# spencerkent/vision-transform-codes

Hardware: AMD Instinct MI355X
Metric: patches/sec through 200-iter FISTA + dict update, 1024-atom dict (higher is better)
Workload: dtype f16x3

## Files before the change

### vision-transform-codes_amd/csrc/fc_fused.hip

```cpp
#include "fc_fused.h"
#include "fused_common.h"

#include <stdlib.h>
#include <mutex>
#include <vector>

namespace vtc {

struct FusedParams {
  const float* images;
  const float* init;
  float* codes;
  const uint4* packA[2];
  const uint4* packT[2];
  const float* betas;
  int64_t b;
  int s;
  int num_iters;
  int fista;
  float eta, cutoff;
  const float* eta_dev;
  float lam;
  const float* dscale;
  unsigned long long* stamps;
// ... 201 lines not shown
  {                                                                         \
    const int j_ = (i) + RING;                                              \
    const int sg_ = (j_ < 16) ? (sg) : (((sg) + 1) % (2 * NPH));            \
    const int i_ = (j_ < 16) ? j_ : j_ - 16;                                \
    _Pragma("unroll") for (int part = 0; part < NP; ++part)                 \
        ring[part][(i) % RING] = VTC_LOAD_SEG(part, sg_, i_);               \
  }

  auto step3 = [&](int p, int buf, bool pipe, int sg, auto&& between) {
    uint4 yb_next[NP];
#pragma unroll
    for (int part = 0; part < NP; ++part)
      yb_next[part] = *reinterpret_cast<const uint4*>(
          Yx + (buf * NP + part) * kYxPart + yx_rd);
#pragma unroll
    for (int ks = 0; ks < 8; ++ks) {
      uint4 yb[NP];
#pragma unroll
      for (int part = 0; part < NP; ++part) {
        yb[part] = yb_next[part];
        if (ks + 1 < 8)
          yb_next[part] = *reinterpret_cast<const uint4*>(
              Yx + (buf * NP + part) * kYxPart + yx_rd + 32 * (ks + 1));
      }
#pragma unroll
      for (int nb = 0; nb < 2; ++nb) {
        const int i = 2 * ks + nb;
        uint4 a[NP];
#pragma unroll
        for (int part = 0; part < NP; ++part)
          a[part] = pipe ? ring[part][i % RING] : VTC_LOAD_T(part, p, nb, ks);
        Racc[nb] = mfma16<F16>(a[0], yb[0], Racc[nb]);
        if constexpr (NP == 2) {
          Racc[nb] = mfma16<F16>(a[0], yb[1], Racc[nb]);
          Racc[nb] = mfma16<F16>(a[1], yb[0], Racc[nb]);
        }
        between(i);
        if (pipe) VTC_REFILL(sg, i)
        __builtin_amdgcn_sched_barrier(0);
      }
    }
  };
  auto nothing = [](int) {};

  auto exchange_r = [&]() {
    float v[2][16];
#pragma unroll
    for (int nb = 0; nb < 2; ++nb)
#pragma unroll
      for (int e = 0; e < 16; ++e) {
        v[nb][e] = sub_rn(Racc[nb][e], Xr[nb][e]);
        if (F16) v[nb][e] *= r_scale;
      }
    if (F16) {
      float m = 0.f;
#pragma unroll
      for (int nb = 0; nb < 2; ++nb)
#pragma unroll
        for (int e = 0; e < 16; ++e) m = fmaxf(m, fabsf(v[nb][e]));
      m = fmaxf(m, __shfl_xor(m, 32, 64));
      float f = 1.f;
      if (xr_calls > 0) {
        const float* prev = Stat + ((xr_calls - 1) & 1) * 128;
        const float Mx = fmaxf(fmaxf(prev[r], prev[32 + r]),
                               fmaxf(prev[64 + r], prev[96 + r]));
        if (Mx > 2048.f && Mx < __builtin_inff())
          f = ldexpf(1.f, 9 - ilogbf(Mx));
      }
      if (h == 0) Stat[(xr_calls & 1) * 128 + w * 32 + r] = m * f;
      ++xr_calls;
      if (__any(f != 1.f)) {
#pragma unroll
        for (int p = 0; p < NPH; ++p)
#pragma unroll
          for (int e = 0; e < 16; ++e) Y[p][e] *= f;
#pragma unroll
        for (int p = 0; p < CR; ++p)
#pragma unroll
          for (int e = 0; e < 16; ++e) Cr[p][e] *= f;
#pragma unroll
        for (int pl = 0; pl < L::CL; ++pl)
#pragma unroll
          for (int g = 0; g < 4; ++g) {
            float4* c4 = reinterpret_cast<float4*>(Cst + cst_ln + pl * 16384 +
                                                   g * 1024);
            float4 c = *c4;
            c.x *= f; c.y *= f; c.z *= f; c.w *= f;
            *c4 = c;
          }
#pragma unroll
        for (int nb = 0; nb < 2; ++nb)
#pragma unroll
          for (int e = 0; e < 16; ++e) {
            Xr[nb][e] *= f;
            v[nb][e] *= f;
          }
        cutoff_l *= f;
        inv_sigma_y *= 1.f / f;
      }
    }
#pragma unroll
    for (int nb = 0; nb < 2; ++nb) {
#pragma unroll
      for (int g = 0; g < 4; ++g) {
        const float v4[4] = {v[nb][4 * g], v[nb][4 * g + 1], v[nb][4 * g + 2],
                             v[nb][4 * g + 3]};
        uint2 hi, lo;
        split_packed<F16, 4, NP == 2>(v4, hi, lo);
        char* dst = Rx + rx_wr + 64 * nb + 16 * g;
        *reinterpret_cast<uint2*>(dst) = hi;
        if (NP == 2) *reinterpret_cast<uint2*>(dst + kRxPart) = lo;
      }
    }
#pragma unroll
    for (int nb = 0; nb < 2; ++nb)
#pragma unroll
      for (int e = 0; e < 16; ++e) Racc[nb][e] = 0.f;
    __syncthreads();
  };

  if (warm) {
#pragma unroll
    for (int p = 0; p < NPH; ++p) {
      publish_y(Y[p], p & 1);
      __syncthreads();
      step3(p, p & 1, false, 0, nothing);
    }
  }
  exchange_r();

#pragma unroll
  for (int i = 0; i < RING; ++i)
#pragma unroll
    for (int part = 0; part < NP; ++part)
      ring[part][i] = VTC_LOAD_SEG(part, 0, i);

  const bool fista = P.fista != 0;
  unsigned long long acc_t[5] = {0, 0, 0, 0, 0};
  unsigned long long t0 = 0, t1 = 0;
#define VTC_STAMP(slot)                    \
  if (STAMP) {                             \
    t1 = stamp_now();                      \
    acc_t[slot] += t1 - t0;                \
    t0 = t1;                               \
  }
  if (STAMP) t0 = stamp_now();

  f32x16 Gb[2];
  float4 cold4;
  float cn4[4];

  auto epilogue_elem = [&](int p, int e, const f32x16& Gp, float beta) {
    const int g = e >> 2, k = e & 3;
    if (MODE == 7) {
      const float cn = Y[p][e] + Gp[e];
      Y[p][e] = cn;
      cn4[k] = cn;
      if (k == 3) {
        if (p < CREG) {
#pragma unroll
          for (int q = 0; q < 4; ++q) Cr[p < CREG ? p : 0][4 * g + q] = cn4[q];
        } else {
          *reinterpret_cast<float4*>(Cst + cst_ln + (p - CREG) * 16384 +
                                     g * 1024) =
              make_float4(cn4[0], cn4[1], cn4[2], cn4[3]);
        }
      }
      return;
    }
    if (k == 0) {
      if (p < CREG) {
        cold4 = make_float4(Cr[p < CREG ? p : 0][4 * g + 0],
                            Cr[p < CREG ? p : 0][4 * g + 1],
                            Cr[p < CREG ? p : 0][4 * g + 2],
                            Cr[p < CREG ? p : 0][4 * g + 3]);
      } else {
        cold4 = *reinterpret_cast<const float4*>(
            Cst + cst_ln + (p - CREG) * 16384 + g * 1024);
      }
    }
    const float co = (k == 0) ? cold4.x : (k == 1) ? cold4.y
                   : (k == 2) ? cold4.z : cold4.w;
    const float c = sub_rn(Y[p][e], mul_rn(eta, Gp[e]));
    const float cn = shrink_fast<MODE>(c, cutoff_l);
    Y[p][e] = fista ? add_rn(cn, mul_rn(beta, sub_rn(cn, co))) : cn;
    cn4[k] = cn;
    if (k == 3) {
      if (p < CREG) {
#pragma unroll
        for (int q = 0; q < 4; ++q) Cr[p < CREG ? p : 0][4 * g + q] = cn4[q];
      } else {
        *reinterpret_cast<float4*>(Cst + cst_ln + (p - CREG) * 16384 +
                                   g * 1024) =
            make_float4(cn4[0], cn4[1], cn4[2], cn4[3]);
      }
      const float v4[4] = {Y[p][4 * g], Y[p][4 * g + 1], Y[p][4 * g + 2],
                           Y[p][4 * g + 3]};
      uint2 hi, lo;
      split_packed<F16, 4, NP == 2>(v4, hi, lo);
      char* dst = Yx + (p & 1) * NP * kYxPart + yx_wr + 16 * g;
      *reinterpret_cast<uint2*>(dst) = hi;
      if (NP == 2) *reinterpret_cast<uint2*>(dst + kYxPart) = lo;
    }
  };

  auto step1 = [&](int p, int sg, bool overlap, float beta) {
    f32x16& G = Gb[p & 1];
#pragma unroll
    for (int e = 0; e < 16; ++e) G[e] = 0.f;
    uint4 rb_next[NP];
#pragma unroll
    for (int part = 0; part < NP; ++part)
      rb_next[part] =
          *reinterpret_cast<const uint4*>(Rx + part * kRxPart + rx_rd);
#pragma unroll
    for (int i = 0; i < 16; ++i) {
      uint4 rb[NP];
#pragma unroll
      for (int part = 0; part < NP; ++part) {
        rb[part] = rb_next[part];
        if (i + 1 < 16)
          rb_next[part] = *reinterpret_cast<const uint4*>(
              Rx + part * kRxPart + rx_rd + 32 * (i + 1));
      }
      G = mfma16<F16>(ring[0][i % RING], rb[0], G);
      if constexpr (NP == 2) {
        G = mfma16<F16>(ring[0][i % RING], rb[1], G);
        G = mfma16<F16>(ring[1][i % RING], rb[0], G);
      }
      if (overlap) {
        epilogue_elem(p - 1, i, Gb[(p - 1) & 1], beta);
        __builtin_amdgcn_sched_barrier(0);
      }
      VTC_REFILL(sg, i)
      __builtin_amdgcn_sched_barrier(0);
    }
  };

  for (int it = 0; it < P.num_iters; ++it) {
    const float beta = fista ? P.betas[it] : 0.f;
    step1(0, 0, false, beta);
    VTC_STAMP(0)
#pragma unroll
    for (int p = 0; p < NPH; ++p) {
      if (p + 1 < NPH) {
        step1(p + 1, 2 * p + 1, true, beta);
        VTC_STAMP(0)
      }
      __syncthreads();
      VTC_STAMP(2)
      if (p + 2 == NPH) {
        step3(p, p & 1, true, 2 * p + 2, [&](int i) {
          epilogue_elem(NPH - 1, i, Gb[(NPH - 1) & 1], beta);
          __builtin_amdgcn_sched_barrier(0);
        });
      } else {
        step3(p, p & 1, true, (p + 1 < NPH) ? 2 * p + 2 : 2 * NPH - 1, nothing);
      }
      VTC_STAMP(3)
    }
    exchange_r();
    VTC_STAMP(4)
  }
  if (STAMP && lane == 0) {
#pragma unroll
    for (int k = 0; k < 5; ++k) atomicAdd(P.stamps + k, acc_t[k]);
    atomicAdd(P.stamps + 7, 1ull);
  }
#undef VTC_STAMP

#pragma unroll
  for (int p = 0; p < NPH; ++p) {
#pragma unroll
    for (int g = 0; g < 4; ++g) {
      float4 v;
      if (p < CREG) {
        v = make_float4(Cr[p < CREG ? p : 0][4 * g + 0],
                        Cr[p < CREG ? p : 0][4 * g + 1],
                        Cr[p < CREG ? p : 0][4 * g + 2],
                        Cr[p < CREG ? p : 0][4 * g + 3]);
      } else {
        v = *reinterpret_cast<const float4*>(Cst + cst_ln +
                                             (p - CREG) * 16384 + g * 1024);
      }
      if (F16) {
        v.x *= inv_sigma_y;
        v.y *= inv_sigma_y;
        v.z *= inv_sigma_y;
        v.w *= inv_sigma_y;
      }
      if (live)
        *reinterpret_cast<float4*>(P.codes + patch * s + kPhaseAtoms * p +
                                   32 * w + 8 * g + 4 * h) = v;
    }
  }
#undef VTC_LOAD_A
#undef VTC_LOAD_T
#undef VTC_LOAD_SEG
#undef VTC_REFILL
#undef VTC_SEG_IS_T
#undef VTC_SEG_PHASE
}

template <int NPH, int NP, int MODE, bool F16 = false, bool STAMP = false>
__global__ __launch_bounds__(256, 1) void fused_fista_kernel16(FusedParams P) {
  static_assert(!F16 || NP == 2, "the f16 split exists as three products only");
  using L = FusedLds<NPH, NP>;
  constexpr int CREG = L::CREG;
  constexpr int CR = CREG > 0 ? CREG : 1;
  constexpr int RING = (NP == 1) ? 16 : 8;
  constexpr int NPROD = (NP == 2) ? 3 : 1;
  extern __shared__ __attribute__((aligned(16))) char smem[];
  char* Cst = smem;
  char* Yx = smem + L::cst_bytes;
  char* Rx = Yx + L::yx_bytes;
  float* Stat = reinterpret_cast<float*>(Rx + L::rx_bytes);

  const int tid = threadIdx.x;
  const int lane = tid & 63;
  const int w = __builtin_amdgcn_readfirstlane(tid >> 6);
  const int c = lane & 15, q = lane >> 4;
  int64_t patch[2];
  bool live[2];
#pragma unroll
  for (int n = 0; n < 2; ++n) {
    patch[n] = (int64_t)blockIdx.x * kFP + 16 * n + c;
    live[n] = patch[n] < P.b;
  }
  const int s = P.s;

  const unsigned pack_bytes_total = (unsigned)s * kFN * 2u;
  const unsigned a_wave_off = (unsigned)w * (16u * 64u * 16u);
  const unsigned t_wave_off = (unsigned)(4 * w) * (4u * 64u * 16u);
  __amdgpu_buffer_rsrc_t rsA[NP], rsT[NP];
#pragma unroll
  for (int part = 0; part < NP; ++part) {
    rsA[part] = __builtin_amdgcn_make_buffer_rsrc(
        (void*)((const char*)P.packA[part] + a_wave_off), 0,
        (int)(pack_bytes_total - a_wave_off), 0x00020000);
    rsT[part] = __builtin_amdgcn_make_buffer_rsrc(
        (void*)((const char*)P.packT[part] + t_wave_off), 0,
        (int)(pack_bytes_total - t_wave_off), 0x00020000);
  }
  const unsigned frag_voff = (unsigned)lane * 16u;
#define VTC_LOAD_A(part, p, i) \
  buffer_load16(rsA[part], frag_voff, (unsigned)(((4 * (p)) * 16 + (i)) * 1024))
#define VTC_LOAD_T(part, p, nb, ks) \
  buffer_load16(rsT[part], frag_voff,  \
                (unsigned)((((p) * 16 + (nb)) * 4 + (ks)) * 1024))

  const int swap = ((c >> 2) ^ (c >> 3)) & 1;
  const int rd_chunk = 32 * (q >> 1) + 16 * ((q & 1) ^ swap);
  const int wr_chunk = 16 * ((q >> 1) ^ swap) + 8 * (q & 1);
  const int yx_rd = c * kYxRow + rd_chunk;
  const int yx_wr = c * kYxRow + 64 * w + wr_chunk;
  const int rx_rd = c * kRxRow + rd_chunk;
  const int rx_wr = c * kRxRow + 128 * w + wr_chunk;
  const int cst_ln = w * 4096 + lane * 16;
  constexpr int kYxHalf = 16 * kYxRow, kRxHalf = 16 * kRxRow;

  f32x16 Y[NPH];
  f32x16 Cr[CR];
  f32x4 Xr[4][2];
  f32x4 Racc[4][2];
  uint4 ring[NP][RING];

#pragma unroll
  for (int nb = 0; nb < 4; ++nb) {
#pragma unroll
    for (int n = 0; n < 2; ++n) {
      float4 v = make_float4(0.f, 0.f, 0.f, 0.f);
      if (live[n])
        v = *reinterpret_cast<const float4*>(P.images + patch[n] * kFN + 64 * w +
                                             16 * nb + 4 * q);
      Xr[nb][n][0] = v.x;
      Xr[nb][n][1] = v.y;
      Xr[nb][n][2] = v.z;
      Xr[nb][n][3] = v.w;
    }
  }
  const bool warm = (P.init != nullptr);
#pragma unroll
  for (int p = 0; p < NPH; ++p) {
#pragma unroll
    for (int g = 0; g < 4; ++g) {
      float4 v = make_float4(0.f, 0.f, 0.f, 0.f);
      if (warm && live[g & 1])
        v = *reinterpret_cast<const float4*>(P.init + patch[g & 1] * s +
                                             kPhaseAtoms * p + 32 * w +
                                             16 * (g >> 1) + 4 * q);
      Y[p][4 * g + 0] = v.x;
      Y[p][4 * g + 1] = v.y;
      Y[p][4 * g + 2] = v.z;
      Y[p][4 * g + 3] = v.w;
    }
  }
  float sigma_y[2] = {1.f, 1.f}, inv_sigma_y[2] = {1.f, 1.f};
  float sigma_d = 1.f, inv_sigma_d = 1.f;
  if (F16) {
    float sx[2] = {0.f, 0.f}, sy[2] = {0.f, 0.f};
#pragma unroll
    for (int nb = 0; nb < 4; ++nb)
#pragma unroll
      for (int n = 0; n < 2; ++n)
#pragma unroll
        for (int k = 0; k < 4; ++k) sx[n] += Xr[nb][n][k] * Xr[nb][n][k];
    if (warm) {
#pragma unroll
      for (int p = 0; p < NPH; ++p)
#pragma unroll
        for (int e = 0; e < 16; ++e) sy[(e >> 2) & 1] += Y[p][e] * Y[p][e];
    }
    float* red = reinterpret_cast<float*>(Rx);
#pragma unroll
    for (int n = 0; n < 2; ++n) {
      sx[n] += __shfl_xor(sx[n], 16, 64);
      sx[n] += __shfl_xor(sx[n], 32, 64);
      sy[n] += __shfl_xor(sy[n], 16, 64);
      sy[n] += __shfl_xor(sy[n], 32, 64);
      if (q == 0) {
        red[w * 64 + 16 * n + c] = sx[n];
        red[w * 64 + 32 + 16 * n + c] = sy[n];
      }
    }
    __syncthreads();
    float m2[2];
#pragma unroll
    for (int n = 0; n < 2; ++n) {
      float tx = 0.f, ty = 0.f;
#pragma unroll
      for (int v = 0; v < 4; ++v) {
        tx += red[v * 64 + 16 * n + c];
        ty += red[v * 64 + 32 + 16 * n + c];
      }
      m2[n] = fmaxf(tx, ty);
    }
    __syncthreads();
    sigma_d = P.dscale[0];
    inv_sigma_d = P.dscale[1];
#pragma unroll
    for (int n = 0; n < 2; ++n) {
      int e2 = 0;
      if (m2[n] > 0.f && m2[n] < __builtin_inff()) e2 = ilogbf(m2[n]) >> 1;
      e2 = e2 < -60 ? -60 : (e2 > 60 ? 60 : e2);
      sigma_y[n] = ldexpf(1.f, 8 - e2);
      inv_sigma_y[n] = ldexpf(1.f, e2 - 8);
      const float sx_scale = sigma_d * sigma_y[n];
#pragma unroll
      for (int nb = 0; nb < 4; ++nb)
#pragma unroll
        for (int k = 0; k < 4; ++k) Xr[nb][n][k] *= sx_scale;
    }
#pragma unroll
    for (int p = 0; p < NPH; ++p)
#pragma unroll
      for (int e = 0; e < 16; ++e) Y[p][e] *= sigma_y[(e >> 2) & 1];
  }
  float eta = P.eta, cutoff = P.cutoff;
  if (P.eta_dev) {
    eta = *P.eta_dev;
    cutoff = mul_rn(P.lam, eta);
  }
  float cutoff_l[2] = {cutoff, cutoff};
  if (F16) {
    eta = eta * (0.5f * inv_sigma_d);
    cutoff_l[0] = cutoff * sigma_y[0];
    cutoff_l[1] = cutoff * sigma_y[1];
  }
  const float r_scale = F16 ? 2.f * inv_sigma_d : 1.f;
  int xr_calls = 0;
#pragma unroll
  for (int p = 0; p < NPH; ++p) {
#pragma unroll
    for (int g = 0; g < 4; ++g) {
      if (p < CREG) {
#pragma unroll
        for (int k = 0; k < 4; ++k)
          Cr[p < CREG ? p : 0][4 * g + k] = Y[p][4 * g + k];
      } else {
        *reinterpret_cast<float4*>(Cst + cst_ln + (p - CREG) * 16384 +
                                   g * 1024) =
            make_float4(Y[p][4 * g + 0], Y[p][4 * g + 1], Y[p][4 * g + 2],
                        Y[p][4 * g + 3]);
      }
    }
  }
#pragma unroll
  for (int nb = 0; nb < 4; ++nb)
#pragma unroll
    for (int n = 0; n < 2; ++n)
#pragma unroll
      for (int k = 0; k < 4; ++k) Racc[nb][n][k] = 0.f;

  auto publish_group = [&](const f32x16& y, int g, int buf) {
    const float v4[4] = {y[4 * g], y[4 * g + 1], y[4 * g + 2], y[4 * g + 3]};
    uint2 hi, lo;
    split_packed<F16, 4, NP == 2>(v4, hi, lo);
    char* dst = Yx + buf * NP * kYxPart + yx_wr + 32 * (g >> 1) +
                kYxHalf * (g & 1);
    *reinterpret_cast<uint2*>(dst) = hi;
    if (NP == 2) *reinterpret_cast<uint2*>(dst + kYxPart) = lo;
  };

#define VTC_SEG_IS_T(sg) (((sg) >= 2 && ((sg) % 2) == 0) || (sg) == 2 * NPH - 1)
#define VTC_SEG_PHASE(sg)                                        \
  ((sg) == 0 ? 0                                                 \
             : (sg) == 2 * NPH - 1 ? NPH - 1                     \
                                   : ((sg) % 2 ? ((sg) + 1) / 2 : (sg) / 2 - 1))
#define VTC_LOAD_SEG(part, sg, i)                                          \
  (VTC_SEG_IS_T(sg) ? VTC_LOAD_T(part, VTC_SEG_PHASE(sg), (i) & 3, (i) >> 2) \
                    : VTC_LOAD_A(part, VTC_SEG_PHASE(sg), (i)))
#define VTC_REFILL(sg, i)                                                   \
  {                                                                         \
    const int j_ = (i) + RING;                                              \
    const int sg_ = (j_ < 16) ? (sg) : (((sg) + 1) % (2 * NPH));            \
    const int i_ = (j_ < 16) ? j_ : j_ - 16;                                \
    _Pragma("unroll") for (int part = 0; part < NP; ++part)                 \
        ring[part][(i) % RING] = VTC_LOAD_SEG(part, sg_, i_);               \
  }
#define VTC_MFMA_PAIR(acc0, acc1, a, b)                                     \
  _Pragma("unroll") for (int prod = 0; prod < NPROD; ++prod) {              \
    acc0 = mfma_k32<F16>(a[prod == 2], b[0][prod == 1], acc0);              \
    acc1 = mfma_k32<F16>(a[prod == 2], b[1][prod == 1], acc1);              \
  }

  auto step3 = [&](int p, int buf, bool pipe, int sg, auto&& between) {
    uint4 yb[2][NP], yb_next[2][NP];
#pragma unroll
    for (int n = 0; n < 2; ++n)
#pragma unroll
      for (int part = 0; part < NP; ++part)
        yb_next[n][part] = *reinterpret_cast<const uint4*>(
            Yx + (buf * NP + part) * kYxPart + yx_rd + kYxHalf * n);
#pragma unroll
    for (int i = 0; i < 16; ++i) {
      const int ks = i >> 2, nb = i & 3;
      if (nb == 0) {
#pragma unroll
        for (int n = 0; n < 2; ++n)
#pragma unroll
          for (int part = 0; part < NP; ++part) yb[n][part] = yb_next[n][part];
      }
      if (nb < 2 && ks + 1 < 4) {
#pragma unroll
        for (int part = 0; part < NP; ++part)
          yb_next[nb][part] = *reinterpret_cast<const uint4*>(
              Yx + (buf * NP + part) * kYxPart + yx_rd + kYxHalf * nb +
              64 * (ks + 1));
      }
      uint4 a[NP];
#pragma unroll
      for (int part = 0; part < NP; ++part)
        a[part] = pipe ? ring[part][i % RING] : VTC_LOAD_T(part, p, nb, ks);
      VTC_MFMA_PAIR(Racc[nb][0], Racc[nb][1], a, yb)
      between(i);
      if (pipe) VTC_REFILL(sg, i)
      __builtin_amdgcn_sched_barrier(0);
    }
  };
  auto nothing = [](int) {};

  auto exchange_r = [&]() {
    float v[4][2][4];
#pragma unroll
    for (int nb = 0; nb < 4; ++nb)
#pragma unroll
      for (int n = 0; n < 2; ++n)
#pragma unroll
        for (int k = 0; k < 4; ++k) {
          v[nb][n][k] = sub_rn(Racc[nb][n][k], Xr[nb][n][k]);
          if (F16) v[nb][n][k] *= r_scale;
        }
    if (F16) {
      float f[2] = {1.f, 1.f};
#pragma unroll
      for (int n = 0; n < 2; ++n) {
        float m = 0.f;
#pragma unroll
        for (int nb = 0; nb < 4; ++nb)
#pragma unroll
          for (int k = 0; k < 4; ++k) m = fmaxf(m, fabsf(v[nb][n][k]));
        m = fmaxf(m, __shfl_xor(m, 16, 64));
        m = fmaxf(m, __shfl_xor(m, 32, 64));
        const int row = 16 * n + c;
        if (xr_calls > 0) {
          const float* prev = Stat + ((xr_calls - 1) & 1) * 128;
          const float Mx = fmaxf(fmaxf(prev[row], prev[32 + row]),
                                 fmaxf(prev[64 + row], prev[96 + row]));
          if (Mx > 2048.f && Mx < __builtin_inff())
            f[n] = ldexpf(1.f, 9 - ilogbf(Mx));
        }
        if (q == 0) Stat[(xr_calls & 1) * 128 + w * 32 + row] = m * f[n];
      }
      ++xr_calls;
      if (__any(f[0] != 1.f || f[1] != 1.f)) {
#pragma unroll
        for (int p = 0; p < NPH; ++p)
#pragma unroll
          for (int e = 0; e < 16; ++e) Y[p][e] *= f[(e >> 2) & 1];
#pragma unroll
        for (int p = 0; p < CR; ++p)
#pragma unroll
          for (int e = 0; e < 16; ++e) Cr[p][e] *= f[(e >> 2) & 1];
#pragma unroll
        for (int pl = 0; pl < L::CL; ++pl)
#pragma unroll
          for (int g = 0; g < 4; ++g) {
            float4* c4 = reinterpret_cast<float4*>(Cst + cst_ln + pl * 16384 +
                                                   g * 1024);
            float4 cc = *c4;
            const float fg = f[g & 1];
            cc.x *= fg; cc.y *= fg; cc.z *= fg; cc.w *= fg;
            *c4 = cc;
          }
#pragma unroll
        for (int n = 0; n < 2; ++n) {
#pragma unroll
          for (int nb = 0; nb < 4; ++nb)
#pragma unroll
            for (int k = 0; k < 4; ++k) {
              Xr[nb][n][k] *= f[n];
              v[nb][n][k] *= f[n];
            }
          cutoff_l[n] *= f[n];
          inv_sigma_y[n] *= 1.f / f[n];
        }
      }
    }
#pragma unroll
    for (int nb = 0; nb < 4; ++nb) {
#pragma unroll
      for (int n = 0; n < 2; ++n) {
        const float v4[4] = {v[nb][n][0], v[nb][n][1], v[nb][n][2], v[nb][n][3]};
        uint2 hi, lo;
        split_packed<F16, 4, NP == 2>(v4, hi, lo);
        char* dst = Rx + rx_wr + 32 * nb + kRxHalf * n;
        *reinterpret_cast<uint2*>(dst) = hi;
        if (NP == 2) *reinterpret_cast<uint2*>(dst + kRxPart) = lo;
      }
    }
#pragma unroll
    for (int nb = 0; nb < 4; ++nb)
#pragma unroll
      for (int n = 0; n < 2; ++n)
#pragma unroll
        for (int k = 0; k < 4; ++k) Racc[nb][n][k] = 0.f;
    __syncthreads();
  };

  if (warm) {
#pragma unroll
    for (int p = 0; p < NPH; ++p) {
#pragma unroll
      for (int g = 0; g < 4; ++g) publish_group(Y[p], g, p & 1);
      __syncthreads();
      step3(p, p & 1, false, 0, nothing);
    }
  }
  exchange_r();

#pragma unroll
  for (int i = 0; i < RING; ++i)
#pragma unroll
    for (int part = 0; part < NP; ++part)
      ring[part][i] = VTC_LOAD_SEG(part, 0, i);

  const bool fista = P.fista != 0;
  unsigned long long acc_t[5] = {0, 0, 0, 0, 0};
  unsigned long long t0 = 0, t1 = 0;
#define VTC_STAMP(slot)                    \
  if (STAMP) {                             \
    t1 = stamp_now();                      \
    acc_t[slot] += t1 - t0;                \
    t0 = t1;                               \
  }
  if (STAMP) t0 = stamp_now();

  f32x4 Gb[2][4];
  float4 cold4;
  float cn4[4];

  auto epilogue_elem = [&](int p, int e, const f32x4 (&Gp)[4], float beta) {
    const int g = e >> 2, k = e & 3;
    if (MODE == 7) {
      const float cn = Y[p][e] + Gp[g][k];
      Y[p][e] = cn;
      cn4[k] = cn;
      if (k == 3) {
        if (p < CREG) {
#pragma unroll
          for (int j = 0; j < 4; ++j) Cr[p < CREG ? p : 0][4 * g + j] = cn4[j];
        } else {
          *reinterpret_cast<float4*>(Cst + cst_ln + (p - CREG) * 16384 +
                                     g * 1024) =
              make_float4(cn4[0], cn4[1], cn4[2], cn4[3]);
        }
      }
      return;
    }
    if (k == 0) {
      if (p < CREG) {
        cold4 = make_float4(Cr[p < CREG ? p : 0][4 * g + 0],
                            Cr[p < CREG ? p : 0][4 * g + 1],
                            Cr[p < CREG ? p : 0][4 * g + 2],
                            Cr[p < CREG ? p : 0][4 * g + 3]);
      } else {
        cold4 = *reinterpret_cast<const float4*>(
            Cst + cst_ln + (p - CREG) * 16384 + g * 1024);
      }
    }
    const float co = (k == 0) ? cold4.x : (k == 1) ? cold4.y
                   : (k == 2) ? cold4.z : cold4.w;
    const float cv = sub_rn(Y[p][e], mul_rn(eta, Gp[g][k]));
    const float cn = shrink_fast<MODE>(cv, cutoff_l[g & 1]);
    Y[p][e] = fista ? add_rn(cn, mul_rn(beta, sub_rn(cn, co))) : cn;
    cn4[k] = cn;
    if (k == 3) {
      if (p < CREG) {
#pragma unroll
        for (int j = 0; j < 4; ++j) Cr[p < CREG ? p : 0][4 * g + j] = cn4[j];
      } else {
        *reinterpret_cast<float4*>(Cst + cst_ln + (p - CREG) * 16384 +
                                   g * 1024) =
            make_float4(cn4[0], cn4[1], cn4[2], cn4[3]);
      }
      publish_group(Y[p], g, p & 1);
    }
  };

  auto step1 = [&](int p, int sg, bool overlap, float beta) {
    f32x4 (&G)[4] = Gb[p & 1];
#pragma unroll
    for (int g = 0; g < 4; ++g)
#pragma unroll
      for (int k = 0; k < 4; ++k) G[g][k] = 0.f;
    uint4 rb[2][NP], rb_next[2][NP];
#pragma unroll
    for (int n = 0; n < 2; ++n)
#pragma unroll
      for (int part = 0; part < NP; ++part)
        rb_next[n][part] = *reinterpret_cast<const uint4*>(
            Rx + part * kRxPart + rx_rd + kRxHalf * n);
#pragma unroll
    for (int i = 0; i < 16; ++i) {
      const int ks = i >> 1, m = i & 1;
      if (m == 0) {
#pragma unroll
        for (int n = 0; n < 2; ++n)
#pragma unroll
          for (int part = 0; part < NP; ++part) rb[n][part] = rb_next[n][part];
      }
      if (ks + 1 < 8) {
#pragma unroll
        for (int part = 0; part < NP; ++part)
          rb_next[m][part] = *reinterpret_cast<const uint4*>(
              Rx + part * kRxPart + rx_rd + kRxHalf * m + 64 * (ks + 1));
      }
      uint4 a[NP];
#pragma unroll
      for (int part = 0; part < NP; ++part) a[part] = ring[part][i % RING];
      VTC_MFMA_PAIR(G[2 * m], G[2 * m + 1], a, rb)
      if (overlap) {
        epilogue_elem(p - 1, i, Gb[(p - 1) & 1], beta);
        __builtin_amdgcn_sched_barrier(0);
      }
      VTC_REFILL(sg, i)
      __builtin_amdgcn_sched_barrier(0);
    }
  };

  for (int it = 0; it < P.num_iters; ++it) {
    const float beta = fista ? P.betas[it] : 0.f;
    step1(0, 0, false, beta);
    VTC_STAMP(0)
#pragma unroll
    for (int p = 0; p < NPH; ++p) {
      if (p + 1 < NPH) {
        step1(p + 1, 2 * p + 1, true, beta);
        VTC_STAMP(0)
      }
      __syncthreads();
      VTC_STAMP(2)
      if (p + 2 == NPH) {
        step3(p, p & 1, true, 2 * p + 2, [&](int i) {
          epilogue_elem(NPH - 1, i, Gb[(NPH - 1) & 1], beta);
          __builtin_amdgcn_sched_barrier(0);
        });
      } else {
        step3(p, p & 1, true, (p + 1 < NPH) ? 2 * p + 2 : 2 * NPH - 1, nothing);
      }
      VTC_STAMP(3)
    }
    exchange_r();
    VTC_STAMP(4)
  }
  if (STAMP && lane == 0) {
#pragma unroll
    for (int k = 0; k < 5; ++k) atomicAdd(P.stamps + k, acc_t[k]);
    atomicAdd(P.stamps + 7, 1ull);
  }
#undef VTC_STAMP

#pragma unroll
  for (int p = 0; p < NPH; ++p) {
#pragma unroll
    for (int g = 0; g < 4; ++g) {
      float4 v;
      if (p < CREG) {
        v = make_float4(Cr[p < CREG ? p : 0][4 * g + 0],
                        Cr[p < CREG ? p : 0][4 * g + 1],
                        Cr[p < CREG ? p : 0][4 * g + 2],
                        Cr[p < CREG ? p : 0][4 * g + 3]);
      } else {
        v = *reinterpret_cast<const float4*>(Cst + cst_ln +
                                             (p - CREG) * 16384 + g * 1024);
      }
      if (F16) {
        v.x *= inv_sigma_y[g & 1];
        v.y *= inv_sigma_y[g & 1];
        v.z *= inv_sigma_y[g & 1];
        v.w *= inv_sigma_y[g & 1];
      }
      if (live[g & 1])
        *reinterpret_cast<float4*>(P.codes + patch[g & 1] * s + kPhaseAtoms * p +
                                   32 * w + 16 * (g >> 1) + 4 * q) = v;
    }
  }
#undef VTC_LOAD_A
#undef VTC_LOAD_T
#undef VTC_LOAD_SEG
#undef VTC_REFILL
#undef VTC_MFMA_PAIR
#undef VTC_SEG_IS_T
#undef VTC_SEG_PHASE
}

}

namespace vtc {

static int phases_for(int64_t s) { return (int)(s / kPhaseAtoms); }

bool fused_shape_supported(int64_t b, int64_t n, int64_t s, int precision) {
  if (n != kFN || b <= 0) return false;
  if (s % kPhaseAtoms != 0) return false;
  const int nph = phases_for(s);
  if (!(nph == 2 || nph == 4 || nph == 8)) return false;
  return precision == VTC_BF16 || precision == VTC_BF16X3 ||
         precision == VTC_F16X3;
}

static int fused_parts(int precision) { return precision == VTC_BF16 ? 1 : 2; }

struct FusedLayout {
  unsigned short* packs[4] = {nullptr, nullptr, nullptr, nullptr};
  float* dscale;
  FusedLayout(Carver& ws, int64_t s, int parts) {
    for (int part = 0; part < parts; ++part) {
      packs[2 * part] = ws.take<unsigned short>((size_t)s * kFN);
      packs[2 * part + 1] = ws.take<unsigned short>((size_t)s * kFN);
    }
    dscale = ws.take<float>(2);
  }
};

size_t fused_workspace_bytes(int64_t b, int64_t n, int64_t s, int precision) {
  if (!fused_shape_supported(b, n, s, precision)) return 256;
  return measured_bytes<FusedLayout>(s, fused_parts(precision));
}

static bool default_tile16(int precision) {
  return precision == VTC_F16X3 || precision == VTC_BF16;
}
static bool use_tile16(int precision) {
  const char* v = getenv("VTC_FUSED_TILE");
  if (v && v[0] == '1' && v[1] == '6' && v[2] == 0) return true;
  if (v && v[0] == '3' && v[1] == '2' && v[2] == 0) return false;
  return default_tile16(precision);
}

template <int NPH, int NP, int MODE, bool F16, bool STAMP, bool TILE16>
static auto fused_kernel() {
  if constexpr (TILE16)
    return fused_fista_kernel16<NPH, NP, MODE, F16, STAMP>;
  else
    return fused_fista_kernel<NPH, NP, MODE, F16, STAMP>;
}

template <int NPH, int NP, int MODE, bool F16, bool TILE16>
static int launch_fused(const FusedParams& P, hipStream_t st) {
  using L = FusedLds<NPH, NP>;
  auto kernel = fused_kernel<NPH, NP, MODE, F16, false, TILE16>();
  static unsigned long long configured = 0;
  if (first_use_on_this_device(&configured)) {
    VTC_HIP_CHECK(hipFuncSetAttribute(
        reinterpret_cast<const void*>(kernel),
        hipFuncAttributeMaxDynamicSharedMemorySize, L::total));
  }
  const unsigned grid = (unsigned)ceil_div(P.b, kFP);
  hipLaunchKernelGGL(kernel, dim3(grid), dim3(256), L::total, st, P);
  VTC_LAUNCH_CHECK();
  return VTC_OK;
}

template <int NPH, int NP, bool F16, bool TILE16>
static int launch_stamped(FusedParams P, hipStream_t st) {
  using L = FusedLds<NPH, NP>;
  static const bool no_epilogue = getenv("VTC_FUSED_NOEPI") != nullptr;
  auto kernel = no_epilogue
                    ? fused_kernel<NPH, NP, 7, F16, true, TILE16>()
                    : fused_kernel<NPH, NP, VTC_SOFT, F16, true, TILE16>();
  unsigned long long* dev = nullptr;
  VTC_HIP_CHECK(hipMalloc(&dev, 8 * sizeof(unsigned long long)));
  VTC_HIP_CHECK(hipMemsetAsync(dev, 0, 8 * sizeof(unsigned long long), st));
  VTC_HIP_CHECK(hipFuncSetAttribute(
      reinterpret_cast<const void*>(kernel),
      hipFuncAttributeMaxDynamicSharedMemorySize, L::total));
  P.stamps = dev;
  hipLaunchKernelGGL(kernel, dim3((unsigned)ceil_div(P.b, kFP)), dim3(256),
                     L::total, st, P);
  VTC_LAUNCH_CHECK();
  unsigned long long host[8];
  VTC_HIP_CHECK(hipMemcpyAsync(host, dev, sizeof(host), hipMemcpyDeviceToHost,
                               st));
  VTC_HIP_CHECK(hipStreamSynchronize(st));
  VTC_HIP_CHECK(hipFree(dev));
  const char* names[5] = {"step1+epi", "epi-alone", "barrier", "step3",
                          "exchange"};
  double total = 0;
  for (int k = 0; k < 5; ++k) total += (double)host[k];
  const double per = (double)host[7] * P.num_iters * NPH;
  for (int k = 0; k < 5; ++k)
    fprintf(stderr, "[vtc stamps] %-9s %5.1f%%  %8.0f cycles/phase/wave\n",
            names[k], 100.0 * host[k] / total, host[k] / per);
  return VTC_OK;
}

template <int NPH, int NP, bool F16, bool TILE16>
static int dispatch_mode(const FusedParams& P, int threshold, hipStream_t st) {
  static const bool stamps = getenv("VTC_FUSED_STAMPS") != nullptr;
  if (stamps && threshold == VTC_SOFT && NPH == 8 && NP == 2)
    return launch_stamped<NPH, NP, F16, TILE16>(P, st);
  switch (threshold) {
    case VTC_SOFT: return launch_fused<NPH, NP, VTC_SOFT, F16, TILE16>(P, st);
    case VTC_SOFT_NONNEG:
      return launch_fused<NPH, NP, VTC_SOFT_NONNEG, F16, TILE16>(P, st);
    case VTC_HARD: return launch_fused<NPH, NP, VTC_HARD, F16, TILE16>(P, st);
    default: return launch_fused<NPH, NP, VTC_HARD_NONNEG, F16, TILE16>(P, st);
  }
}

template <int NP, bool F16, bool TILE16>
static int dispatch_phases(const FusedParams& P, int threshold,
                           hipStream_t st) {
  switch (phases_for(P.s)) {
    case 2: return dispatch_mode<2, NP, F16, TILE16>(P, threshold, st);
    case 4: return dispatch_mode<4, NP, F16, TILE16>(P, threshold, st);
    case 8: return dispatch_mode<8, NP, F16, TILE16>(P, threshold, st);
  }
  set_error("fused FISTA: unsupported atom count %d", P.s);
  return VTC_ERR_UNSUPPORTED;
}

constexpr int kBetaTable = 16384;
const float* fista_beta_table_on_this_device() {
  static float* tables[64] = {nullptr};
  static std::mutex guard;
  int dev = 0;
  if (hipGetDevice(&dev) != hipSuccess || dev < 0 || dev > 63) return nullptr;
  std::lock_guard<std::mutex> lock(guard);
  if (tables[dev]) return tables[dev];
  std::vector<float> host;
  fista_betas(kBetaTable, &host);
  float* table = nullptr;
  if (hipMalloc(&table, sizeof(float) * kBetaTable) != hipSuccess)
    return nullptr;
  if (hipMemcpy(table, host.data(), sizeof(float) * kBetaTable,
                hipMemcpyHostToDevice) != hipSuccess) {
    (void)hipFree(table);
    return nullptr;
  }
  tables[dev] = table;
  return table;
}

int fused_max_iters() { return kBetaTable; }

int run_fused(const float* images, const float* dictionary,
              const float* initial_codes, float* codes, int64_t b, int64_t n,
              int64_t s, float eta, const float* eta_dev,
              float sparsity_weight, int num_iters, int variant,
              int threshold, int precision, void* workspace,
              size_t workspace_bytes, int* iters_run, hipStream_t st) {
  if (!fused_shape_supported(b, n, s, precision)) {
    set_error("fused FISTA: unsupported shape");
    return VTC_ERR_UNSUPPORTED;
  }
  if (num_iters > kBetaTable) {
    set_error("fused FISTA: at most %d iterations per call", kBetaTable);
    return VTC_ERR_UNSUPPORTED;
  }
  if (!workspace ||
      workspace_bytes < fused_workspace_bytes(b, n, s, precision)) {
    set_error("fused FISTA: workspace too small");
    return VTC_ERR_WORKSPACE;
  }
  const float* betas_dev = fista_beta_table_on_this_device();
  if (!betas_dev) {
    set_error("fused FISTA: could not place the momentum table on the device");
    return VTC_ERR_HIP;
  }
  const int parts = fused_parts(precision);
  const bool f16 = (precision == VTC_F16X3);
  Carver ws(workspace);
  FusedParams P;
  const FusedLayout L(ws, s, parts);
  unsigned short* const* packs = L.packs;
  float* dscale = L.dscale;
  if (f16) {
    hipLaunchKernelGGL(dictionary_scale_kernel, dim3(1), dim3(1024), 0, st,
                       dictionary, (int64_t)s * kFN, dscale);
    VTC_LAUNCH_CHECK();
  }
  const bool tile16 = use_tile16(precision);
  auto pack = f16 ? (tile16 ? pack_dictionary_kernel<true, true>
                            : pack_dictionary_kernel<true, false>)
                  : (tile16 ? pack_dictionary_kernel<false, true>
                            : pack_dictionary_kernel<false, false>);
  hipLaunchKernelGGL(pack, dim3(256), dim3(256), 0, st, dictionary, (int)s,
                     packs[0], packs[1], packs[2], packs[3], dscale);
  VTC_LAUNCH_CHECK();
  P.images = images;
  P.init = initial_codes;
  P.codes = codes;
  for (int part = 0; part < 2; ++part) {
    P.packA[part] = reinterpret_cast<const uint4*>(packs[2 * (part % parts)]);
    P.packT[part] =
        reinterpret_cast<const uint4*>(packs[2 * (part % parts) + 1]);
  }
  P.betas = betas_dev;
  P.b = b;
  P.s = (int)s;
  P.num_iters = num_iters;
  P.fista = (variant == VTC_FISTA) ? 1 : 0;
  P.eta = eta;
  P.eta_dev = eta_dev;
  P.lam = sparsity_weight;
  P.cutoff = sparsity_weight * eta;
  P.dscale = dscale;
  P.stamps = nullptr;
  int rc;
  if (tile16)
    rc = f16          ? dispatch_phases<2, true, true>(P, threshold, st)
         : parts == 2 ? dispatch_phases<2, false, true>(P, threshold, st)
                      : dispatch_phases<1, false, true>(P, threshold, st);
  else
    rc = f16          ? dispatch_phases<2, true, false>(P, threshold, st)
         : parts == 2 ? dispatch_phases<2, false, false>(P, threshold, st)
                      : dispatch_phases<1, false, false>(P, threshold, st);
  if (rc == VTC_OK && iters_run) *iters_run = num_iters;
  return rc;
}

}

extern "C" int vtc_init(void) {
  if (!vtc::fista_beta_table_on_this_device()) {
    vtc::set_error("vtc_init: could not place the momentum table on the device");
    return VTC_ERR_HIP;
  }
  return VTC_OK;
}
```

Before: 1.701 million.

## Add schedule variants spreading FISTA epilogue across MFMA phases and overlapping residual exchange

Adds a SCHED template parameter with two bits. SPREAD splits the per-phase shrink/momentum epilogue into two half-stages and interleaves them with the MFMAs of both step1 and the previous step3, so epilogue ALU work is hidden behind matrix ops instead of sitting on the critical path. EARLY_R reorders the last transpose segment block-major so part of the residual exchange can start inside the final step3. The default picks SPREAD for f16 and single-part variants, selectable via VTC_FUSED_SCHED. This adds instantiations and register pressure, and could disturb existing instruction scheduling.

```diff
diff --git a/vision-transform-codes_amd/csrc/fc_fused.hip b/vision-transform-codes_amd/csrc/fc_fused.hip
--- a/vision-transform-codes_amd/csrc/fc_fused.hip
+++ b/vision-transform-codes_amd/csrc/fc_fused.hip
@@ -527,9 +527,13 @@
 #undef VTC_SEG_PHASE
 }
 
-template <int NPH, int NP, int MODE, bool F16 = false, bool STAMP = false>
+template <int NPH, int NP, int MODE, bool F16 = false, bool STAMP = false,
+          int SCHED = 0>
 __global__ __launch_bounds__(256, 1) void fused_fista_kernel16(FusedParams P) {
   static_assert(!F16 || NP == 2, "the f16 split exists as three products only");
+  static_assert(SCHED >= 0 && SCHED < 4, "two schedule bits");
+  constexpr bool SPREAD = (SCHED & 1) != 0 && NPH > 2;
+  constexpr bool EARLY_R = (SCHED & 2) != 0;
   using L = FusedLds<NPH, NP>;
   constexpr int CREG = L::CREG;
   constexpr int CR = CREG > 0 ? CREG : 1;
@@ -732,8 +736,13 @@
   ((sg) == 0 ? 0                                                 \
              : (sg) == 2 * NPH - 1 ? NPH - 1                     \
                                    : ((sg) % 2 ? ((sg) + 1) / 2 : (sg) / 2 - 1))
+#define VTC_SEG_BLOCK_MAJOR(sg) (EARLY_R && (sg) == 2 * NPH - 1)
+#define VTC_T_NB(sg, i) \
+  (VTC_SEG_BLOCK_MAJOR(sg) ? 2 * ((i) >> 3) + ((i) & 1) : (i) & 3)
+#define VTC_T_KS(sg, i) (VTC_SEG_BLOCK_MAJOR(sg) ? ((i) >> 1) & 3 : (i) >> 2)
 #define VTC_LOAD_SEG(part, sg, i)                                          \
-  (VTC_SEG_IS_T(sg) ? VTC_LOAD_T(part, VTC_SEG_PHASE(sg), (i) & 3, (i) >> 2) \
+  (VTC_SEG_IS_T(sg) ? VTC_LOAD_T(part, VTC_SEG_PHASE(sg), VTC_T_NB(sg, i), \
+                                 VTC_T_KS(sg, i))                          \
                     : VTC_LOAD_A(part, VTC_SEG_PHASE(sg), (i)))
 #define VTC_REFILL(sg, i)                                                   \
   {                                                                         \
@@ -873,6 +882,138 @@
     __syncthreads();
   };
 
+  float xf[2] = {1.f, 1.f}, xm[2] = {0.f, 0.f};
+  auto exchange_guard = [&]() {
+#pragma unroll
+    for (int n = 0; n < 2; ++n) {
+      xf[n] = 1.f;
+      xm[n] = 0.f;
+      if (F16 && xr_calls > 0) {
+        const int row = 16 * n + c;
+        const float* prev = Stat + ((xr_calls - 1) & 1) * 128;
+        const float Mx = fmaxf(fmaxf(prev[row], prev[32 + row]),
+                               fmaxf(prev[64 + row], prev[96 + row]));
+        if (Mx > 2048.f && Mx < __builtin_inff())
+          xf[n] = ldexpf(1.f, 9 - ilogbf(Mx));
+      }
+    }
+  };
+  float xv[4];
+  auto exchange_block_a = [&](int nb, int n) {
+#pragma unroll
+    for (int k = 0; k < 4; ++k) {
+      xv[k] = sub_rn(Racc[nb][n][k], Xr[nb][n][k]);
+      if (F16) {
+        xv[k] *= r_scale;
+        xm[n] = fmaxf(xm[n], fabsf(xv[k]));
+        xv[k] *= xf[n];
+      }
+      Racc[nb][n][k] = 0.f;
+    }
+  };
+  auto exchange_block_b = [&](int nb, int n) {
+    uint2 hi, lo;
+    split_packed<F16, 4, NP == 2>(xv, hi, lo);
+    char* dst = Rx + rx_wr + 32 * nb + kRxHalf * n;
+    *reinterpret_cast<uint2*>(dst) = hi;
+    if (NP == 2) *reinterpret_cast<uint2*>(dst + kRxPart) = lo;
+  };
+  auto exchange_block = [&](int nb, int n) {
+    exchange_block_a(nb, n);
+    exchange_block_b(nb, n);
+  };
+  auto exchange_finish = [&](int nb0) {
+#pragma unroll
+    for (int nb = nb0; nb < 4; ++nb)
+#pragma unroll
+      for (int n = 0; n < 2; ++n) exchange_block(nb, n);
+    if (F16) {
+#pragma unroll
+      for (int n = 0; n < 2; ++n) {
+        float m = xm[n];
+        m = fmaxf(m, __shfl_xor(m, 16, 64));
+        m = fmaxf(m, __shfl_xor(m, 32, 64));
+        if (q == 0) Stat[(xr_calls & 1) * 128 + w * 32 + 16 * n + c] = m * xf[n];
+      }
+      ++xr_calls;
+      if (__any(xf[0] != 1.f || xf[1] != 1.f)) {
+#pragma unroll
+        for (int p = 0; p < NPH; ++p)
+#pragma unroll
+          for (int e = 0; e < 16; ++e) Y[p][e] *= xf[(e >> 2) & 1];
+#pragma unroll
+        for (int p = 0; p < CR; ++p)
+#pragma unroll
+          for (int e = 0; e < 16; ++e) Cr[p][e] *= xf[(e >> 2) & 1];
+#pragma unroll
+        for (int pl = 0; pl < L::CL; ++pl)
+#pragma unroll
+          for (int g = 0; g < 4; ++g) {
+            float4* c4 = reinterpret_cast<float4*>(Cst + cst_ln + pl * 16384 +
+                                                   g * 1024);
+            float4 cc = *c4;
+            const float fg = xf[g & 1];
+            cc.x *= fg; cc.y *= fg; cc.z *= fg; cc.w *= fg;
+            *c4 = cc;
+          }
+#pragma unroll
+        for (int n = 0; n < 2; ++n) {
+#pragma unroll
+          for (int nb = 0; nb < 4; ++nb)
+#pragma unroll
+            for (int k = 0; k < 4; ++k) Xr[nb][n][k] *= xf[n];
+          cutoff_l[n] *= xf[n];
+          inv_sigma_y[n] *= 1.f / xf[n];
+        }
+      }
+    }
+    __syncthreads();
+  };
+
+  auto step3_last = [&](int buf, int sg) {
+    uint4 yb[2][NP], yb_next[2][NP];
+#pragma unroll
+    for (int n = 0; n < 2; ++n)
+#pragma unroll
+      for (int part = 0; part < NP; ++part)
+        yb_next[n][part] = *reinterpret_cast<const uint4*>(
+            Yx + (buf * NP + part) * kYxPart + yx_rd + kYxHalf * n);
+#pragma unroll
+    for (int i = 0; i < 16; ++i) {
+      const int j = i & 1, nb = VTC_T_NB(sg, i);
+      if (j == 0) {
+#pragma unroll
+        for (int n = 0; n < 2; ++n)
+#pragma unroll
+          for (int part = 0; part < NP; ++part) yb[n][part] = yb_next[n][part];
+      }
+      if (i + 2 < 16) {
+#pragma unroll
+        for (int part = 0; part < NP; ++part)
+          yb_next[j][part] = *reinterpret_cast<const uint4*>(
+              Yx + (buf * NP + part) * kYxPart + yx_rd + kYxHalf * j +
+              64 * VTC_T_KS(sg, i + 2));
+      }
+      uint4 a[NP];
+#pragma unroll
+      for (int part = 0; part < NP; ++part) a[part] = ring[part][i % RING];
+      VTC_MFMA_PAIR(Racc[nb][0], Racc[nb][1], a, yb)
+      if (i == 6) {
+        exchange_guard();
+        __builtin_amdgcn_sched_barrier(0);
+      }
+      if (i >= 8) {
+        if (j == 0)
+          exchange_block_a((i - 8) >> 2, ((i - 8) >> 1) & 1);
+        else
+          exchange_block_b((i - 8) >> 2, ((i - 8) >> 1) & 1);
+        __builtin_amdgcn_sched_barrier(0);
+      }
+      VTC_REFILL(sg, i)
+      __builtin_amdgcn_sched_barrier(0);
+    }
+  };
+
   if (warm) {
 #pragma unroll
     for (int p = 0; p < NPH; ++p) {
@@ -952,8 +1093,57 @@
       publish_group(Y[p], g, p & 1);
     }
   };
-
-  auto step1 = [&](int p, int sg, bool overlap, float beta) {
+  auto epilogue_stage_a = [&](int p, int e, const f32x4 (&Gp)[4]) {
+    const int g = e >> 2, k = e & 3;
+    if (MODE == 7) {
+      cn4[k] = Y[p][e] + Gp[g][k];
+      return;
+    }
+    if (k == 0) {
+      if (p < CREG) {
+        cold4 = make_float4(Cr[p < CREG ? p : 0][4 * g + 0],
+                            Cr[p < CREG ? p : 0][4 * g + 1],
+                            Cr[p < CREG ? p : 0][4 * g + 2],
+                            Cr[p < CREG ? p : 0][4 * g + 3]);
+      } else {
+        cold4 = *reinterpret_cast<const float4*>(
+            Cst + cst_ln + (p - CREG) * 16384 + g * 1024);
+      }
+    }
+    const float cv = sub_rn(Y[p][e], mul_rn(eta, Gp[g][k]));
+    cn4[k] = shrink_fast<MODE>(cv, cutoff_l[g & 1]);
+  };
+  auto epilogue_stage_b = [&](int p, int e, float beta) {
+    const int g = e >> 2, k = e & 3;
+    const float cn = cn4[k];
+    if (MODE == 7) {
+      Y[p][e] = cn;
+    } else {
+      const float co = (k == 0) ? cold4.x : (k == 1) ? cold4.y
+                     : (k == 2) ? cold4.z : cold4.w;
+      Y[p][e] = fista ? add_rn(cn, mul_rn(beta, sub_rn(cn, co))) : cn;
+    }
+    if (k == 3) {
+      if (p < CREG) {
+#pragma unroll
+        for (int j = 0; j < 4; ++j) Cr[p < CREG ? p : 0][4 * g + j] = cn4[j];
+      } else {
+        *reinterpret_cast<float4*>(Cst + cst_ln + (p - CREG) * 16384 +
+                                   g * 1024) =
+            make_float4(cn4[0], cn4[1], cn4[2], cn4[3]);
+      }
+      if (MODE != 7) publish_group(Y[p], g, p & 1);
+    }
+  };
+  auto epilogue_half = [&](int p, int e0, int i, const f32x4 (&Gp)[4],
+                           float beta) {
+    if ((i & 1) == 0)
+      epilogue_stage_a(p, e0 + (i >> 1), Gp);
+    else
+      epilogue_stage_b(p, e0 + (i >> 1), beta);
+  };
+
+  auto step1 = [&](int p, int sg, int overlap, float beta) {
     f32x4 (&G)[4] = Gb[p & 1];
 #pragma unroll
     for (int g = 0; g < 4; ++g)
@@ -985,9 +1175,12 @@
 #pragma unroll
       for (int part = 0; part < NP; ++part) a[part] = ring[part][i % RING];
       VTC_MFMA_PAIR(G[2 * m], G[2 * m + 1], a, rb)
-      if (overlap) {
+      if (overlap == 1) {
         epilogue_elem(p - 1, i, Gb[(p - 1) & 1], beta);
         __builtin_amdgcn_sched_barrier(0);
+      } else if (overlap == 2) {
+        epilogue_half(p - 1, 8, i, Gb[(p - 1) & 1], beta);
+        __builtin_amdgcn_sched_barrier(0);
       }
       VTC_REFILL(sg, i)
       __builtin_amdgcn_sched_barrier(0);
@@ -996,12 +1189,12 @@
 
   for (int it = 0; it < P.num_iters; ++it) {
     const float beta = fista ? P.betas[it] : 0.f;
-    step1(0, 0, false, beta);
+    step1(0, 0, 0, beta);
     VTC_STAMP(0)
 #pragma unroll
     for (int p = 0; p < NPH; ++p) {
       if (p + 1 < NPH) {
-        step1(p + 1, 2 * p + 1, true, beta);
+        step1(p + 1, 2 * p + 1, (SPREAD && p > 0) ? 2 : 1, beta);
         VTC_STAMP(0)
       }
       __syncthreads();
@@ -1011,12 +1204,22 @@
           epilogue_elem(NPH - 1, i, Gb[(NPH - 1) & 1], beta);
           __builtin_amdgcn_sched_barrier(0);
         });
+      } else if (SPREAD && p + 2 < NPH) {
+        step3(p, p & 1, true, 2 * p + 2, [&](int i) {
+          epilogue_half(p + 1, 0, i, Gb[(p + 1) & 1], beta);
+          __builtin_amdgcn_sched_barrier(0);
+        });
+      } else if (EARLY_R && p + 1 == NPH) {
+        step3_last(p & 1, 2 * NPH - 1);
       } else {
         step3(p, p & 1, true, (p + 1 < NPH) ? 2 * p + 2 : 2 * NPH - 1, nothing);
       }
       VTC_STAMP(3)
     }
-    exchange_r();
+    if (EARLY_R)
+      exchange_finish(2);
+    else
+      exchange_r();
     VTC_STAMP(4)
   }
   if (STAMP && lane == 0) {
@@ -1058,6 +1261,9 @@
 #undef VTC_MFMA_PAIR
 #undef VTC_SEG_IS_T
 #undef VTC_SEG_PHASE
+#undef VTC_SEG_BLOCK_MAJOR
+#undef VTC_T_NB
+#undef VTC_T_KS
 }
 
 }
@@ -1104,18 +1310,32 @@
   return default_tile16(precision);
 }
 
-template <int NPH, int NP, int MODE, bool F16, bool STAMP, bool TILE16>
+template <int NP, bool F16>
+constexpr int default_sched() {
+  return (F16 || NP == 1) ? 1 : 0;
+}
+static int use_sched(int by_default) {
+  const char* v = getenv("VTC_FUSED_SCHED");
+  if (v && v[0] >= '0' && v[0] <= '3' && v[1] == 0) return v[0] - '0';
+  return by_default;
+}
+
+template <int NPH, int NP, int MODE, bool F16, bool STAMP, bool TILE16,
+          int SCHED>
 static auto fused_kernel() {
-  if constexpr (TILE16)
+  static_assert(TILE16 || SCHED == 0, "schedules exist on the 16x16x32 tile");
+  if constexpr (TILE16 && SCHED != 0)
+    return fused_fista_kernel16<NPH, NP, MODE, F16, STAMP, SCHED>;
+  else if constexpr (TILE16)
     return fused_fista_kernel16<NPH, NP, MODE, F16, STAMP>;
   else
     return fused_fista_kernel<NPH, NP, MODE, F16, STAMP>;
 }
 
-template <int NPH, int NP, int MODE, bool F16, bool TILE16>
+template <int NPH, int NP, int MODE, bool F16, bool TILE16, int SCHED>
 static int launch_fused(const FusedParams& P, hipStream_t st) {
   using L = FusedLds<NPH, NP>;
-  auto kernel = fused_kernel<NPH, NP, MODE, F16, false, TILE16>();
+  auto kernel = fused_kernel<NPH, NP, MODE, F16, false, TILE16, SCHED>();
   static unsigned long long configured = 0;
   if (first_use_on_this_device(&configured)) {
     VTC_HIP_CHECK(hipFuncSetAttribute(
@@ -1128,13 +1348,14 @@
   return VTC_OK;
 }
 
-template <int NPH, int NP, bool F16, bool TILE16>
+template <int NPH, int NP, bool F16, bool TILE16, int SCHED>
 static int launch_stamped(FusedParams P, hipStream_t st) {
   using L = FusedLds<NPH, NP>;
   static const bool no_epilogue = getenv("VTC_FUSED_NOEPI") != nullptr;
-  auto kernel = no_epilogue
-                    ? fused_kernel<NPH, NP, 7, F16, true, TILE16>()
-                    : fused_kernel<NPH, NP, VTC_SOFT, F16, true, TILE16>();
+  auto kernel =
+      no_epilogue
+          ? fused_kernel<NPH, NP, 7, F16, true, TILE16, SCHED>()
+          : fused_kernel<NPH, NP, VTC_SOFT, F16, true, TILE16, SCHED>();
   unsigned long long* dev = nullptr;
   VTC_HIP_CHECK(hipMalloc(&dev, 8 * sizeof(unsigned long long)));
   VTC_HIP_CHECK(hipMemsetAsync(dev, 0, 8 * sizeof(unsigned long long), st));
@@ -1161,27 +1382,49 @@
   return VTC_OK;
 }
 
-template <int NPH, int NP, bool F16, bool TILE16>
+template <int NPH, int NP, bool F16, bool TILE16, int SCHED>
 static int dispatch_mode(const FusedParams& P, int threshold, hipStream_t st) {
   static const bool stamps = getenv("VTC_FUSED_STAMPS") != nullptr;
-  if (stamps && threshold == VTC_SOFT && NPH == 8 && NP == 2)
-    return launch_stamped<NPH, NP, F16, TILE16>(P, st);
+  if constexpr (SCHED == 0 || (NPH == 8 && NP == 2)) {
+    if (stamps && threshold == VTC_SOFT && NPH == 8 && NP == 2)
+      return launch_stamped<NPH, NP, F16, TILE16, SCHED>(P, st);
+  }
   switch (threshold) {
-    case VTC_SOFT: return launch_fused<NPH, NP, VTC_SOFT, F16, TILE16>(P, st);
+    case VTC_SOFT:
+      return launch_fused<NPH, NP, VTC_SOFT, F16, TILE16, SCHED>(P, st);
     case VTC_SOFT_NONNEG:
-      return launch_fused<NPH, NP, VTC_SOFT_NONNEG, F16, TILE16>(P, st);
-    case VTC_HARD: return launch_fused<NPH, NP, VTC_HARD, F16, TILE16>(P, st);
-    default: return launch_fused<NPH, NP, VTC_HARD_NONNEG, F16, TILE16>(P, st);
-  }
+      return launch_fused<NPH, NP, VTC_SOFT_NONNEG, F16, TILE16, SCHED>(P, st);
+    case VTC_HARD:
+      return launch_fused<NPH, NP, VTC_HARD, F16, TILE16, SCHED>(P, st);
+    default:
+      return launch_fused<NPH, NP, VTC_HARD_NONNEG, F16, TILE16, SCHED>(P, st);
+  }
+}
+
+template <int NPH, int NP, bool F16, bool TILE16>
+static int dispatch_sched(const FusedParams& P, int threshold,
+                          hipStream_t st) {
+  if constexpr (TILE16) {
+    const int sched = use_sched(default_sched<NP, F16>());
+    if constexpr (NPH > 2) {
+      if (sched == 1)
+        return dispatch_mode<NPH, NP, F16, TILE16, 1>(P, threshold, st);
+      if (sched == 3)
+        return dispatch_mode<NPH, NP, F16, TILE16, 3>(P, threshold, st);
+    }
+    if (sched & 2)
+      return dispatch_mode<NPH, NP, F16, TILE16, 2>(P, threshold, st);
+  }
+  return dispatch_mode<NPH, NP, F16, TILE16, 0>(P, threshold, st);
 }
 
 template <int NP, bool F16, bool TILE16>
 static int dispatch_phases(const FusedParams& P, int threshold,
                            hipStream_t st) {
   switch (phases_for(P.s)) {
-    case 2: return dispatch_mode<2, NP, F16, TILE16>(P, threshold, st);
-    case 4: return dispatch_mode<4, NP, F16, TILE16>(P, threshold, st);
-    case 8: return dispatch_mode<8, NP, F16, TILE16>(P, threshold, st);
+    case 2: return dispatch_sched<2, NP, F16, TILE16>(P, threshold, st);
+    case 4: return dispatch_sched<4, NP, F16, TILE16>(P, threshold, st);
+    case 8: return dispatch_sched<8, NP, F16, TILE16>(P, threshold, st);
   }
   set_error("fused FISTA: unsupported atom count %d", P.s);
   return VTC_ERR_UNSUPPORTED;
```

New measurement: 1.720 million (median of 6 runs). +1.1%, better.
